# ariel415el/SoundEventDetection-Pytorch

Measured on AMD Instinct MI355X. Metric: SED train clips/sec (60s,64-mel,9-layer CNN), higher is better.
Workload: dtype bf16; 1 GPU; Cnn_AvgPooling main widths [32, 64, 128, 128], 60 s / 32 kHz / 64-mel clips (T=6001 frames, NFFT 1024, hop 320), batch 32/GPU, train step = waveform->log-mel->fwd->BCE->bwd->Adam-amsgrad; frontend_constants=bench, graph_replay=False, global_batch=32, frames=6001, parallelism=dp1, frontend_in_step=True, frontend_overlapped=False, frontend_overlap_mode=0, sync_bn=False, rccl_group=False, collectives_executed=False

## Files before the change

soundeventdetection-pytorch_amd/csrc/conv_common.h:

```cpp
#pragma once
#include "common.h"

#include <stdlib.h>

template <typename T> __device__ __forceinline__ int swz(int col);
template <> __device__ __forceinline__ int swz<bf16_t>(int col) { return ((col >> 2) & 3) << 3; }
template <> __device__ __forceinline__ int swz<float>(int col) { return col & 31; }

template <typename T> struct Raw8;
template <> struct Raw8<bf16_t> { bf16x8 v; };
template <> struct Raw8<float> { f32x4 a, b; };
template <typename T> __device__ __forceinline__ Raw8<T> raw_load8(const T* p);
template <> __device__ __forceinline__ Raw8<bf16_t> raw_load8<bf16_t>(const bf16_t* p) {
    Raw8<bf16_t> r; r.v = *reinterpret_cast<const bf16x8*>(p); return r;
}
template <> __device__ __forceinline__ Raw8<float> raw_load8<float>(const float* p) {
    Raw8<float> r;
    r.a = *reinterpret_cast<const f32x4*>(p);
    r.b = *reinterpret_cast<const f32x4*>(p + 4);
    return r;
}
__device__ __forceinline__ void raw_to_f(const Raw8<bf16_t>& r, float (&v)[8]) {
#pragma unroll
    for (int i = 0; i < 8; ++i) v[i] = (float)r.v[i];
}
__device__ __forceinline__ void raw_to_f(const Raw8<float>& r, float (&v)[8]) {
#pragma unroll
    for (int i = 0; i < 4; ++i) { v[i] = r.a[i]; v[4 + i] = r.b[i]; }
}

typedef __attribute__((ext_vector_type(4))) unsigned u32x4;
typedef __attribute__((ext_vector_type(2))) unsigned u32x2;
#define SED_OOB 0x80000000u

__device__ __forceinline__ __amdgpu_buffer_rsrc_t make_srd(const void* base, size_t bytes) {
    return __builtin_amdgcn_make_buffer_rsrc(const_cast<void*>(base), 0, (int)(bytes > 0xFFFFFFFFull ? 0xFFFFFFFFu : (unsigned)bytes),
                                             0x00020000);
}
template <typename T> __device__ __forceinline__ Raw8<T> buf_load8(__amdgpu_buffer_rsrc_t r, unsigned voff);
template <> __device__ __forceinline__ Raw8<bf16_t> buf_load8<bf16_t>(__amdgpu_buffer_rsrc_t r, unsigned voff) {
    Raw8<bf16_t> o;
    o.v = __builtin_bit_cast(bf16x8, __builtin_amdgcn_raw_buffer_load_b128(r, voff, 0, 0));
    return o;
}
template <> __device__ __forceinline__ Raw8<float> buf_load8<float>(__amdgpu_buffer_rsrc_t r, unsigned voff) {
    Raw8<float> o;
    o.a = __builtin_bit_cast(f32x4, __builtin_amdgcn_raw_buffer_load_b128(r, voff, 0, 0));
    o.b = __builtin_bit_cast(f32x4, __builtin_amdgcn_raw_buffer_load_b128(r, voff + 16, 0, 0));
    return o;
}
template <typename T> __device__ __forceinline__ void buf_store8(__amdgpu_buffer_rsrc_t r, unsigned voff, const float (&v)[8]);
template <> __device__ __forceinline__ void buf_store8<bf16_t>(__amdgpu_buffer_rsrc_t r, unsigned voff, const float (&v)[8]) {
    bf16x8 a;
#pragma unroll
    for (int i = 0; i < 8; ++i) a[i] = (bf16_t)v[i];
    __builtin_amdgcn_raw_buffer_store_b128(__builtin_bit_cast(u32x4, a), r, voff, 0, 0);
}
template <> __device__ __forceinline__ void buf_store8<float>(__amdgpu_buffer_rsrc_t r, unsigned voff, const float (&v)[8]) {
    f32x4 a, b;
#pragma unroll
    for (int i = 0; i < 4; ++i) { a[i] = v[i]; b[i] = v[4 + i]; }
    __builtin_amdgcn_raw_buffer_store_b128(__builtin_bit_cast(u32x4, a), r, voff, 0, 0);
    __builtin_amdgcn_raw_buffer_store_b128(__builtin_bit_cast(u32x4, b), r, voff + 16, 0, 0);
}
template <typename T> __device__ __forceinline__ void buf_store4(__amdgpu_buffer_rsrc_t r, unsigned voff, const float (&v)[4]);
template <> __device__ __forceinline__ void buf_store4<bf16_t>(__amdgpu_buffer_rsrc_t r, unsigned voff, const float (&v)[4]) {
    bf16x4 a;
#pragma unroll
    for (int i = 0; i < 4; ++i) a[i] = (bf16_t)v[i];
    __builtin_amdgcn_raw_buffer_store_b64(__builtin_bit_cast(u32x2, a), r, voff, 0, 0);
}
template <> __device__ __forceinline__ void buf_store4<float>(__amdgpu_buffer_rsrc_t r, unsigned voff, const float (&v)[4]) {
    f32x4 a;
#pragma unroll
    for (int i = 0; i < 4; ++i) a[i] = v[i];
    __builtin_amdgcn_raw_buffer_store_b128(__builtin_bit_cast(u32x4, a), r, voff, 0, 0);
}
template <typename T> __device__ __forceinline__ void buf_load4(__amdgpu_buffer_rsrc_t r, unsigned voff, float (&v)[4]);
template <> __device__ __forceinline__ void buf_load4<bf16_t>(__amdgpu_buffer_rsrc_t r, unsigned voff, float (&v)[4]) {
    const bf16x4 a = __builtin_bit_cast(bf16x4, __builtin_amdgcn_raw_buffer_load_b64(r, voff, 0, 0));
#pragma unroll
    for (int i = 0; i < 4; ++i) v[i] = (float)a[i];
}
template <> __device__ __forceinline__ void buf_load4<float>(__amdgpu_buffer_rsrc_t r, unsigned voff, float (&v)[4]) {
    const f32x4 a = __builtin_bit_cast(f32x4, __builtin_amdgcn_raw_buffer_load_b128(r, voff, 0, 0));
#pragma unroll
    for (int i = 0; i < 4; ++i) v[i] = a[i];
}
template <typename T> __device__ __forceinline__ void lds_store_raw(T* dst, const Raw8<T>& r);
template <> __device__ __forceinline__ void lds_store_raw<bf16_t>(bf16_t* dst, const Raw8<bf16_t>& r) {
    *reinterpret_cast<bf16x8*>(dst) = r.v;
}
template <> __device__ __forceinline__ void lds_store_raw<float>(float* dst, const Raw8<float>& r) {
    *reinterpret_cast<f32x4*>(dst) = r.a;
    *reinterpret_cast<f32x4*>(dst + 4) = r.b;
}

template <typename T, int W, int ROWS, int WP, int NTHR, int PS>
struct HaloPlan {
    static constexpr int ITEMS = ROWS * (W + 2) * 4;
    static constexpr int IPT = (ITEMS + NTHR - 1) / NTHR;
    unsigned voff[IPT];
    int lds[IPT];
    unsigned colmask;
    Raw8<T> raw[IPT];

    __device__ __forceinline__ void init(int tid, int Cinp) {
        const int cq = tid & 3;
        colmask = 0;
#pragma unroll
        for (int u = 0; u < IPT; ++u) {
            const int it = tid + u * NTHR;
            const int pix = it >> 2;
            const int rowi = pix / (W + 2), coli = pix - rowi * (W + 2);
            const bool ok = (it < ITEMS) && coli >= 1 && coli <= W;
            voff[u] = ok ? (unsigned)(((rowi * W + coli) * Cinp + cq * 8) * (int)sizeof(T)) : SED_OOB;
            if (ok) colmask |= 1u << u;
            if constexpr (sizeof(T) == 2) lds[u] = (rowi * WP + coli) * PS + ((PS == 32) ? ((cq * 8) ^ swz<T>(coli)) : cq * 8);
            else lds[u] = (rowi * WP + coli) * PS;
        }
    }
    __device__ __forceinline__ void issue(__amdgpu_buffer_rsrc_t img, unsigned tile_off) {
#pragma unroll
        for (int u = 0; u < IPT; ++u) raw[u] = buf_load8<T>(img, voff[u] + tile_off);
    }
    template <int PRO>
    __device__ __forceinline__ void commit(T* __restrict__ xs, int tid, const float* __restrict__ pro_scale,
                                           const float* __restrict__ pro_shift, int c0, int row_lo, int row_hi) const {
        const int cq = tid & 3;
        float sc[8], sh[8];
        if (PRO == SED_PRO_BNRELU) {
#pragma unroll
            for (int e = 0; e < 8; ++e) { sc[e] = pro_scale[c0 + cq * 8 + e]; sh[e] = pro_shift[c0 + cq * 8 + e]; }
        }
        const bool boundary = (row_lo > 0) || (row_hi < ROWS - 1);
#pragma unroll
        for (int u = 0; u < IPT; ++u) {
            const int it = tid + u * NTHR;
            if (u == IPT - 1 && it >= ITEMS) break;
            if constexpr (sizeof(T) == 2) {
                if (PRO == SED_PRO_NONE) {
                    lds_store_raw<T>(xs + lds[u], raw[u]);
                } else {
                    float v[8];
                    raw_to_f(raw[u], v);
                    bool keep = (colmask >> u) & 1;
                    if (boundary) {
                        const int rowi = (it >> 2) / (W + 2);
                        keep = keep && rowi >= row_lo && rowi <= row_hi;
                    }
#pragma unroll
                    for (int e = 0; e < 8; ++e) v[e] = keep ? fmaxf(0.f, fmaf(v[e], sc[e], sh[e])) : 0.f;
                    store8<T>(xs + lds[u], v);
                }
            } else {
                float v[8];
                raw_to_f(raw[u], v);
                const int pix = it >> 2;
                const int rowi = pix / (W + 2), coli = pix - rowi * (W + 2);
                const bool keep = ((colmask >> u) & 1) && rowi >= row_lo && rowi <= row_hi;
                if (PRO == SED_PRO_BNRELU) {
#pragma unroll
                    for (int e = 0; e < 8; ++e) v[e] = keep ? fmaxf(0.f, fmaf(v[e], sc[e], sh[e])) : 0.f;
                }
                const int sx = swz<T>(coli);
#pragma unroll
                for (int e = 0; e < 8; ++e) xs[lds[u] + ((cq * 8 + e) ^ sx)] = v[e];
            }
        }
    }
};


typedef __attribute__((ext_vector_type(4))) short s16x4;
typedef __attribute__((ext_vector_type(8))) short s16x8;
__device__ __forceinline__ s16x4 ds_read_tr16_b64(const bf16_t* p) {
    typedef __attribute__((address_space(3))) s16x4 lds_s16x4;
    return __builtin_amdgcn_ds_read_tr16_b64_v4i16((lds_s16x4*)(const __attribute__((address_space(3))) void*)p);
}
__device__ __forceinline__ bf16x8 join_tr(const s16x4& lo, const s16x4& hi) {
    return __builtin_bit_cast(bf16x8, __builtin_shufflevector(lo, hi, 0, 1, 2, 3, 4, 5, 6, 7));
}


#ifndef SED_BOUNDARY_BRANCH
#define SED_BOUNDARY_BRANCH 1
#endif

enum { DZ_GIVEN = 0, DZ_POOL = 1, DZ_BN = 2 };

struct Wgrad2Params {
    const void* x;
    const float* pro_scale;
    const float* pro_shift;
    const void* dz;
    const void* zsrc;
    const float* scale;
    const float* shift;
    const float* ca;
    const float* cb;
    const float* cc;
    void* dz_out;
    float* ws;
    int B, H, Cinp, Coutp;
    int tilesPerImg, totalTiles, tpb, strips;
    int pro, pool;
    const float* c1_x;
    const float* c1_mean;
    const float* c1_std;
    const float* c1_w;
    int dbg;
    unsigned tpi_M, tpi_l;
    int dzexp;
};


int wgrad3_strips(int B, int H, int W, int Cinp, int Coutp);
int launch_wgrad3(int dzmode, Wgrad2Params& p, int W, hipStream_t st);
int wgrad_wide_strips(int B, int H, int W, int Cinp, int Coutp);
int launch_wgrad_wide(int dzmode, Wgrad2Params& p, int W, hipStream_t st);
int reduce_wgrad_slabs(const float* ws, float* dwpack, int slabs, size_t n, float* dw, int Cout, int Cin, int Cinp, int Coutp, hipStream_t st);

static inline bool sed_w_specialised(int W) { return W == 8 || W == 16 || W == 32 || W == 64; }

#ifdef SED_DEBUG_SWITCHES
#define SED_DBG(p, bit) ((p).dbg & (bit))
#define SED_SET_PRIO(x) set_wave_prio(x)
#else
#define SED_DBG(p, bit) 0
#define SED_SET_PRIO(x) ((void)0)
#endif
static inline int sed_dbg_env() { const char* d = sed_getenv("SED_DBG"); return d ? atoi(d) : 0; }

__device__ __forceinline__ void set_wave_prio(int pr) {
    switch (pr & 3) {
        case 1: __builtin_amdgcn_s_setprio(1); break;
        case 2: __builtin_amdgcn_s_setprio(2); break;
        case 3: __builtin_amdgcn_s_setprio(3); break;
        default: break;
    }
}


struct ConvParams {
    const void* x;
    const float* pro_scale;
    const float* pro_shift;
    const void* wpack;
    void* z;
    const void* zref;
    const float* epi_scale;
    const float* epi_shift;
    const float* epi_mean;
    const float* epi_invstd;
    float* partial;
    int B, H, Cinp, Coutp;
    int tilesPerImg, totalTiles, tpb, nparts;
    int pro, epi;
    int wres;
    const float* c1_x;
    const float* c1_mean;
    const float* c1_std;
    const float* c1_w;
    void* c1_mask;
    int dbg;
    int col_only;
    const unsigned char* cnt;
    int* flag;
    int dry;
    const void* dz_g;
    const float* dz_ca;
    const float* dz_cb;
    const float* dz_cc;
    const float* dz_sc;
    const float* dz_sh;
    void* dz_out;
    int dz_pool;
    unsigned tpi_M, tpi_l, nch_M, nch_l;
    int xexp;
};
inline void sed_fastdiv_make(unsigned d, unsigned* M, unsigned* l) {
    unsigned ll = 0;
    while ((1ull << ll) < d) ++ll;
    *l = ll;
    *M = (unsigned)((((1ull << ll) - d) << 32) / d + 1);
}
__device__ __forceinline__ int sed_fastdiv(int n, unsigned M, unsigned l) { return (int)((__umulhi((unsigned)n, M) + (unsigned)n) >> l); }

int launch_conv_x3(int half, ConvParams& p, int W, hipStream_t st);
int launch_conv_x3pc(ConvParams& p, int W, hipStream_t st);
int launch_wgrad_x3pc(int dzmode, Wgrad2Params& p, int W, hipStream_t st);
int launch_wgrad_x3(int half, int dzmode, Wgrad2Params& p, int W, int wn, hipStream_t st);

int launch_conv_anyw(int dtype, ConvParams& p, int W, hipStream_t st);
int launch_wgrad_anyw(int dtype, int dzmode, Wgrad2Params& p, int W, hipStream_t st);

int launch_conv_pc(ConvParams& p, int W, hipStream_t st);
int launch_conv_wir(ConvParams& p, int W, hipStream_t st);
int launch_conv_w4(ConvParams& p, int W, hipStream_t st);

struct BwdFusedParams {
    const void* x;
    const float* pro_scale;
    const float* pro_shift;
    const void* gsrc;
    const void* zsrc;
    const float* scale;
    const float* shift;
    const float* ca;
    const float* cb;
    const float* cc;
    const void* wpack_t;
    void* dx;
    const void* zref;
    const unsigned char* cnt;
    const float* epi_scale;
    const float* epi_shift;
    const float* epi_mean;
    const float* epi_invstd;
    float* partial;
    int* flag;
    float* ws;
    int B, H, Cinp, Coutp;
    int pool, dzmode, pro, epi;
    int nparts, nwg, tilesPerImg, totalTiles, tpb;
    int dry;
    int prio;
    int abl;
};
int bwd_fused_nwg(int B, int H, int W, int Cinp, int Coutp, int dzmode, int pro, int epi);
int launch_bwd_fused(BwdFusedParams& p, int W, hipStream_t st);
int bwd_fused_max_nwg(int B, int H, int W, int Cinp, int Coutp);
int bwd_fused_c1_nwg(int B, int H);
int bwd_fused_cs_nstrips(int B, int H, int W, int Cinp, int Coutp, int dzmode, int pro, int epi, int pool);
int launch_bwd_fused_cs(BwdFusedParams& p, int W, hipStream_t st);

int launch_bwd_fused_c1(const float* x1, const float* fmean, const float* fstd, const float* w1, const float* sc1, const float* sh1,
                        const void* dy, const void* z2, const float* sc2, const float* sh2, const float* ca, const float* cb,
                        const float* cc, const void* wpack_t, float* a_part, int nparts, float* ws, int B, int H,
                        int* nwg, hipStream_t st);

enum { SED_PRO_C1 = 2, SED_EPI_RELUBWD_C1 = 3 };
enum { SED_PRO_DZBN = 11, SED_PRO_DZPOOL = 12 };

struct C1Ctx {
    float w[9][8];
    float mu[3], is[3];
};
__device__ __forceinline__ void c1ctx_init(C1Ctx& c, const float* __restrict__ w1, int ch0, const float* __restrict__ fmean,
                                           const float* __restrict__ fstd, int col, int W) {
#pragma unroll
    for (int k = 0; k < 9; ++k)
#pragma unroll
        for (int e = 0; e < 8; ++e) c.w[k][e] = w1[(ch0 + e) * 9 + k];
#pragma unroll
    for (int j = 0; j < 3; ++j) {
        const int cc = col + j - 1;
        const bool ok = cc >= 0 && cc < W;
        c.mu[j] = (ok && fmean) ? fmean[cc] : 0.f;
        c.is[j] = ok ? (fstd ? 1.0f / fstd[cc] : 1.0f) : 0.f;
    }
}
__device__ __forceinline__ void c1_norm_row(const C1Ctx& c, const float (&raw)[3], bool row_ok, float (&xn)[3]) {
#pragma unroll
    for (int j = 0; j < 3; ++j) xn[j] = row_ok ? (raw[j] - c.mu[j]) * c.is[j] : 0.f;
}
__device__ __forceinline__ void c1_eval(const C1Ctx& c, const float (&r0)[3], const float (&r1)[3], const float (&r2)[3],
                                        float (&z)[8]) {
#pragma unroll
    for (int e = 0; e < 8; ++e) z[e] = 0.f;
#pragma unroll
    for (int j = 0; j < 3; ++j)
#pragma unroll
        for (int e = 0; e < 8; ++e) z[e] = fmaf(r0[j], c.w[j][e], z[e]);
#pragma unroll
    for (int j = 0; j < 3; ++j)
#pragma unroll
        for (int e = 0; e < 8; ++e) z[e] = fmaf(r1[j], c.w[3 + j][e], z[e]);
#pragma unroll
    for (int j = 0; j < 3; ++j)
#pragma unroll
        for (int e = 0; e < 8; ++e) z[e] = fmaf(r2[j], c.w[6 + j][e], z[e]);
}
__device__ __forceinline__ float buf_load_f32(__amdgpu_buffer_rsrc_t r, unsigned voff) {
    return __builtin_bit_cast(float, __builtin_amdgcn_raw_buffer_load_b32(r, voff, 0, 0));
}

struct C1Mma {
    bf16x8 wa;
};
__device__ __forceinline__ void c1mma_init(C1Mma& m, const float* __restrict__ w1, const float* __restrict__ scale,
                                           const float* __restrict__ shift, int lane) {
    const int ch = lane & 31, g = lane >> 5;
    const float sc = scale[ch], sh = shift[ch];
    const bf16_t sh_hi = (bf16_t)sh;
    const bf16_t sh_lo = (bf16_t)(sh - (float)sh_hi);
#pragma unroll
    for (int j = 0; j < 8; ++j) {
        const int row = 2 * g + (j >> 2), dx = j & 3;
        m.wa[j] = (row < 3 && dx < 3) ? (bf16_t)(w1[ch * 9 + 3 * row + dx] * sc) : (row == 3 && dx == 0) ? sh_hi : (row == 3 && dx == 1) ? sh_lo : (bf16_t)0.f;
    }
}
template <int XW>
__device__ __forceinline__ bf16x8 c1mma_patch_f(const float* __restrict__ xt, int rr, int half, int lane) {
    const int col = half * 32 + (lane & 31), g = lane >> 5;
    const float* p0 = xt + (rr + 2 * g) * XW + col;
    float v[8];
#pragma unroll
    for (int t = 0; t < 3; ++t) { v[t] = p0[t]; v[4 + t] = p0[XW + t]; }
    v[3] = 0.f; v[7] = 0.f;
    bf16x8 xb;
#pragma unroll
    for (int j = 0; j < 8; ++j) xb[j] = (bf16_t)v[j];
    u32x4 xw = __builtin_bit_cast(u32x4, xb);
    xw[2] = g ? 0x3F803F80u : xw[2];
    xw[3] = g ? 0u : xw[3];
    return __builtin_bit_cast(bf16x8, xw);
}
typedef unsigned c1_u32x2_a4 __attribute__((ext_vector_type(2), aligned(4)));
template <int W, int R>
struct C1Tile {
    static constexpr int XP = W + 8;
    static constexpr int XB = ((R * XP / 2 + 15) / 32 * 32 + 16) * 2 >= R * XP ? ((R * XP / 2 + 15) / 32 * 32 + 16) * 2 : ((R * XP / 2 + 15) / 32 * 32 + 48) * 2;
    static constexpr int N = XB + R * XP;
    static_assert(XB >= R * XP && (XB / 2) % 32 == 16 && XP % 2 == 0, "copy B offset");
};
template <int W, int R>
__device__ __forceinline__ void c1tile_lane_offsets(int half, int lane, int& o1, int& o2) {
    typedef C1Tile<W, R> TL;
    const int p = half * 32 + (lane & 31), g = lane >> 5;
    const int src = (p & 1) ? TL::XB + p - 1 : p;
    o1 = src + (g ? 2 * TL::XP : 0);
    o2 = g ? TL::XP + W + 4 : TL::XP + src;
}
__device__ __forceinline__ bf16x8 c1mma_patch_b(const bf16_t* __restrict__ row_rr, int o1, int o2) {
    const c1_u32x2_a4 lo = *reinterpret_cast<const c1_u32x2_a4*>(row_rr + o1);
    const c1_u32x2_a4 hi = *reinterpret_cast<const c1_u32x2_a4*>(row_rr + o2);
    const u32x4 xw = {lo[0], lo[1], hi[0], hi[1]};
    return __builtin_bit_cast(bf16x8, xw);
}
template <int W, int R>
__device__ __forceinline__ void c1tile_init(bf16_t* __restrict__ t, int tid, int nthr) {
    typedef C1Tile<W, R> TL;
    unsigned* w = reinterpret_cast<unsigned*>(t);
    for (int i = tid; i < TL::N / 2; i += nthr) {
        const int e = 2 * i, r = e / TL::XP, c = e - r * TL::XP;
        w[i] = (e < R * TL::XP && c == W + 4) ? 0x3F803F80u : 0u;
    }
}
template <int W, int R>
__device__ __forceinline__ void c1tile_store(bf16_t* __restrict__ t, int r, int c, float x) {
    typedef C1Tile<W, R> TL;
    const bf16_t b = (bf16_t)x;
    t[r * TL::XP + c] = b;
    if (c >= 1) t[TL::XB + r * TL::XP + c - 1] = b;
}
template <int XW, bool WANT_MASK>
__device__ __forceinline__ void c1mma_block(const C1Mma& m, const float* __restrict__ xt, int rr, int half, int lane,
                                            float (&a)[16], unsigned& mask) {
    const bf16x8 xb = c1mma_patch_f<XW>(xt, rr, half, lane);
    f32x16 d;
#pragma unroll
    for (int i = 0; i < 16; ++i) d[i] = 0.f;
    d = __builtin_amdgcn_mfma_f32_32x32x16_bf16(m.wa, xb, d, 0, 0, 0);
    mask = 0;
#pragma unroll
    for (int i = 15; i >= 0; --i) {
        const float y = d[i];
        a[i] = fmaxf(0.f, y);
        if (WANT_MASK)
            asm volatile("v_cmp_lt_f32 vcc, 0, %1\n\tv_addc_co_u32 %0, vcc, %0, %0, vcc" : "+v"(mask) : "v"(y) : "vcc");
    }
}

template <int XW>
__device__ __forceinline__ f32x16 c1mma_block_mfma(const C1Mma& m, const float* __restrict__ xt, int rr, int half, int lane) {
    const bf16x8 xb = c1mma_patch_f<XW>(xt, rr, half, lane);
    f32x16 d;
#pragma unroll
    for (int i = 0; i < 16; ++i) d[i] = 0.f;
    return __builtin_amdgcn_mfma_f32_32x32x16_bf16(m.wa, xb, d, 0, 0, 0);
}
__device__ __forceinline__ f32x16 c1mma_block_mfma_b(const C1Mma& m, const bf16_t* __restrict__ row_rr, int o1, int o2) {
    const bf16x8 xb = c1mma_patch_b(row_rr, o1, o2);
    f32x16 d;
#pragma unroll
    for (int i = 0; i < 16; ++i) d[i] = 0.f;
    return __builtin_amdgcn_mfma_f32_32x32x16_bf16(m.wa, xb, d, 0, 0, 0);
}
template <bool WANT_MASK>
__device__ __forceinline__ void c1mma_block_tail_pk(const f32x16& d, unsigned (&w)[8], unsigned& mask) {
    unsigned mlo = 0, mhi = 0;
    const unsigned one2 = 0x00010001u;
#pragma unroll
    for (int k = 0; k < 8; ++k) {
        const f32x2 r = {d[2 * k], d[2 * k + 1]};
        const bf16x2 rb = __builtin_convertvector(r, bf16x2);
        sed_i16x2 ri = __builtin_bit_cast(sed_i16x2, rb);
        ri = __builtin_elementwise_max(ri, (sed_i16x2){0, 0});
        w[k] = __builtin_bit_cast(unsigned, ri);
        if (WANT_MASK) {
            unsigned t;
            asm("v_pk_min_u16 %0, %1, %2" : "=v"(t) : "v"(w[k]), "v"(one2));
            const unsigned wt = (1u << ((2 * k) & 7)) | (1u << (16 + ((2 * k + 1) & 7)));
            if (k < 4) mlo = __builtin_amdgcn_udot4(t, wt, mlo, false);
            else mhi = __builtin_amdgcn_udot4(t, wt, mhi, false);
        }
    }
    mask = mlo | (mhi << 8);
}
template <bool WANT_MASK>
__device__ __forceinline__ void c1mma_block_tail(const C1Mma& m, const f32x16& d, float (&a)[16], unsigned& mask) {
    mask = 0;
#pragma unroll
    for (int i = 15; i >= 0; --i) {
        const float y = d[i];
        a[i] = fmaxf(0.f, y);
        if (WANT_MASK)
            asm volatile("v_cmp_lt_f32 vcc, 0, %1\n\tv_addc_co_u32 %0, vcc, %0, %0, vcc" : "+v"(mask) : "v"(y) : "vcc");
    }
}
```

soundeventdetection-pytorch_amd/csrc/sed_conv_pc.hip:

```cpp
#include "conv_common.h"

#include <stdlib.h>


namespace {

#ifdef SED_STAMPS
constexpr bool kStamps = true;
#else
constexpr bool kStamps = false;
#endif

constexpr int kPcBlocks = 256;

__device__ __forceinline__ void wg_barrier() {
    asm volatile("s_waitcnt lgkmcnt(0)\n\ts_barrier" ::: "memory");
}

__device__ __forceinline__ int xswz(int col) { return (col >> 2) & 3; }
__device__ __forceinline__ f32x16 zero16() {
    f32x16 z;
#pragma unroll
    for (int i = 0; i < 16; ++i) z[i] = 0.f;
    return z;
// ... 791 lines not shown
        constexpr bool WREGS = C1PRO && NT == 1 && !COL && SED_PC_WREGS;
        bf16x8 wreg[WREGS ? 18 : 1];
        if constexpr (WREGS) {
            const T* __restrict__ wgl = reinterpret_cast<const T*>(p.wpack);
#pragma unroll
            for (int k = 0; k < 18; ++k) {
                const int tap = k >> 1, ks = k & 1;
                wreg[k] = *reinterpret_cast<const bf16x8*>(wgl + ((size_t)(tap * 4 + ks * 2 + hh) * Coutp + n0 + r) * 8);
            }
        }
        auto compute = [&](const T* __restrict__ xsb, const T* __restrict__ wsc, bool first) {
            if (SED_DBG(p, 2)) return;
            if constexpr (WREGS) {
                bf16x8 xf[3][2];
                auto ldx = [&](int k, bf16x8 (&xd)[2]) {
                    const int tap = k >> 1, ks = k & 1, ti = tap / 3, tj = tap % 3;
#pragma unroll
                    for (int mt = 0; mt < 2; ++mt)
                        xd[mt] = *reinterpret_cast<const bf16x8*>(xsb + xoff[mt][tj][ks] + (ti * WP + tj) * 32);
                };
                ldx(0, xf[0]);
                ldx(1, xf[1]);
#pragma unroll
                for (int k = 0; k < 18; ++k) {
                    if (k + 2 < 18) ldx(k + 2, xf[(k + 2) % 3]);
                    __builtin_amdgcn_sched_barrier(0);
#pragma unroll
                    for (int mt = 0; mt < 2; ++mt) acc[mt][0] = mfma(wreg[k], xf[k % 3][mt], acc[mt][0]);
                    __builtin_amdgcn_sched_barrier(0);
                }
                return;
            }
            constexpr int RD = 3;
            bf16x8 xf[RD][2], wf[RD][NT];
            auto ld = [&](int k, bf16x8 (&xd)[2], bf16x8 (&wd)[NT]) {
                const int tap = k >> 1, ks = k & 1, ti = tap / 3, tj = tap % 3;
#pragma unroll
                for (int mt = 0; mt < 2; ++mt)
                    xd[mt] = *reinterpret_cast<const bf16x8*>(xsb + xoff[mt][tj][ks] + (ti * WP + tj) * 32);
#pragma unroll
                for (int nt = 0; nt < NT; ++nt)
                    wd[nt] = *reinterpret_cast<const bf16x8*>(wsc + woff + ((tap * 4 + ks * 2) * BN + nt * 32) * 8);
            };
            constexpr int NK = COL ? 6 : 18;
            auto kmap = [](int s2) { return COL ? (s2 >> 1) * 6 + 2 + (s2 & 1) : s2; };
#pragma unroll
            for (int k = 0; k < RD - 1 && k < NK; ++k) ld(kmap(k), xf[k], wf[k]);
#pragma unroll
            for (int k = 0; k < NK; ++k) {
                if (k + RD - 1 < NK) ld(kmap(k + RD - 1), xf[(k + RD - 1) % RD], wf[(k + RD - 1) % RD]);
                __builtin_amdgcn_sched_barrier(0);
#pragma unroll
                for (int nt = 0; nt < NT; ++nt)
#pragma unroll
                    for (int mt = 0; mt < 2; ++mt) {
                        if (SED_PC_ZEROC && k == 0) {
                            if (first) { asm volatile("" ::: "memory"); acc[mt][nt] = mfma(wf[k % RD][nt], xf[k % RD][mt], zero16()); }
                            else acc[mt][nt] = mfma(wf[k % RD][nt], xf[k % RD][mt], acc[mt][nt]);
                        } else {
                            acc[mt][nt] = mfma(wf[k % RD][nt], xf[k % RD][mt], acc[mt][nt]);
                        }
                    }
                __builtin_amdgcn_sched_barrier(0);
            }
        };

        if (C1PRO && !BLD) build_c1(0, wave, std::integral_constant<int, 0>{});

        unsigned long long tc[4] = {0, 0, 0, 0};
        auto stamp = [&]() -> unsigned long long { return kStamps ? __builtin_amdgcn_s_memtime() : 0ull; };
        auto citer = [&](int j, const T* __restrict__ xsb) {
            const unsigned long long c0 = stamp();
            wg_barrier();
            const unsigned long long c1 = stamp();
            tc[0] += c1 - c0;
            if (C1PRO && j >= nst) return;
            if (j >= nst) return;
            if constexpr (kSplitBuild) build_c1_issue(j + 1, wave);
            constexpr bool ONECH = C1PRO && SED_PC_ONECH;
            const int tl = ONECH ? j : DIV_NCH(j), kc = ONECH ? 0 : j - tl * nchunks;
            if (ONECH || (!SED_PC_ZEROC && kc == 0)) {
#pragma unroll
                for (int mt = 0; mt < 2; ++mt)
#pragma unroll
                    for (int nt = 0; nt < NT; ++nt)
#pragma unroll
                        for (int i = 0; i < 16; ++i) acc[mt][nt][i] = 0.f;
            }
            compute(xsb, ws + (wres ? kc : (j & 1)) * WS, kc == 0);
            const unsigned long long c2 = stamp();
            tc[1] += c2 - c1;
            if (!ONECH && kc != nchunks - 1) return;
            T* osb = os + (nos == 2 ? (tl & 1) : 0) * OSZ;
            if (!(SED_DBG(p, 128)))
#pragma unroll
            for (int mt = 0; mt < 2; ++mt)
#pragma unroll
                for (int nt = 0; nt < NT; ++nt)
#pragma unroll
                    for (int g = 0; g < 4; ++g) {
                        float v[4];
#pragma unroll
                        for (int e = 0; e < 4; ++e) v[e] = acc[mt][nt][4 * g + e];
                        store4<T>(osb + ostg[mt] + nt * 32 + 8 * g, v);
                    }
            const unsigned long long c3 = stamp();
            if constexpr (kSplitBuild) build_c1_finish(j + 1, wave);
            else if (C1PRO && !BLD) build_c1(j + 1, wave, std::integral_constant<int, C1SHARE ? (SED_C1_SHARE == 2 ? 3 : 1) : 0>{});
            if constexpr (CSTAT) {
                const int tile = t_begin + tl;
                const int b_ = DIV_TPI(tile), h0_ = (tile - b_ * p.tilesPerImg) * TH;
                bf16x8 ones;
#pragma unroll
                for (int e = 0; e < 8; ++e) ones[e] = (bf16_t)1.0f;
#pragma unroll
                for (int mt = 0; mt < 2; ++mt) {
                    const int q0s = (wave * 2 + mt) * 32;
                    if (h0_ + q0s / W < H) {
#pragma unroll
                        for (int ks = 0; ks < 2; ++ks) {
                            const T* fp = osb + (q0s + 16 * ks) * BNP;
                            const bf16x8 f = join_tr(ds_read_tr16_b64(fp + offS[0]), ds_read_tr16_b64(fp + offS[1]));
                            gacc = mfma(f, f, gacc);
                            sacc = mfma(ones, f, sacc);
                        }
                    }
                }
            }
            if (kStamps) { tc[2] += c3 - c2; tc[3] += stamp() - c3; }
        };
        for (int j = 0; j < NI; j += 2) {
            citer(j, xs0);
            citer(j + 1, xs0 + XS);
        }
        if (kStamps && (SED_DBG(p, 16)) && blockIdx.x == 8 && lane == 0 && wave == 1)
            printf("pc consumer wave %d: %d stages; cycles barrier %llu kloop %llu staging %llu c1build %llu\n", wave, NI, tc[0], tc[1], tc[2], tc[3]);
        if constexpr (CSTAT) {
            const int idx = 4 * (r >> 3) + (r & 3);
            float dg = 0.f;
#pragma unroll
            for (int i = 0; i < 16; ++i) dg = (i == idx) ? gacc[i] : dg;
            S[0] = sacc[0];
            Q[0] = dg;
        }
        }
    }

    if (EPI != SED_EPI_STORE) {
        __syncthreads();
        float* red = reinterpret_cast<float*>(smem);
        if constexpr (CSTAT) {
            if (wave < 4) {
                const int r_ = lane & 31, hh_ = lane >> 5;
                if (hh_ == 0) red[(wave * 2 + 0) * 32 + r_] = S[0];
                if (hh_ == ((r_ >> 2) & 1)) red[(wave * 2 + 1) * 32 + r_] = Q[0];
            }
        } else
        if (wave >= 4 && wave < 4 + NPW) {
            const int pt = tid - 256;
#pragma unroll
            for (int e = 0; e < 8; ++e) { red[pt * 16 + e] = S[e]; red[pt * 16 + 8 + e] = Q[e]; }
        }
        __syncthreads();
        if (tid < 2 * BN) {
            const int stat = tid / BN, cn = tid % BN;
            const int cg = cn >> 3, e = cn & 7;
            float tot = 0.f;
            if constexpr (CSTAT) {
                for (int w = 0; w < 4; ++w) tot += red[(w * 2 + stat) * 32 + cn];
            } else
            for (int k = 0; k < FQS; ++k) tot += red[(cg + IPR * k) * 16 + stat * 8 + e];
            if (EPI == SED_EPI_RELUBWD && stat) tot *= p.epi_invstd[n0 + cn];
            if constexpr (PSTATS) {
                float sraw = tot;
                if (stat) {
                    sraw = 0.f;
                    for (int k = 0; k < FQS; ++k) sraw += red[(cg + IPR * k) * 16 + e];
                }
                const float sc = p.epi_scale[n0 + cn], is = p.epi_invstd[n0 + cn];
                const float beta = fmaf(p.epi_mean[n0 + cn], sc, p.epi_shift[n0 + cn]);
                const bool ill = fabsf(beta) * is > 8.0f * fabsf(sc);
                if (!stat) {
                    tot = 0.25f * sraw;
                } else if (sc != 0.f && !ill) {
                    tot = (tot - 0.25f * beta * sraw) * (is / sc);
                } else {
                    if (tot != 0.f || sraw != 0.f) atomicOr(p.flag, 1);
                    tot = 0.f;
                }
            }
            p.partial[((size_t)bx * 2 + stat) * Coutp + n0 + cn] = tot;
            for (int row = bx + nbx; row < p.nparts; row += nbx) p.partial[((size_t)row * 2 + stat) * Coutp + n0 + cn] = 0.f;
        }
    }
}

template <int W, int BN, int PRO, int EPI, bool COL = false, int NPW = 4, bool BLD = false, bool WR = false>
int launch_pc_n(ConvParams& p, hipStream_t st) {
    constexpr int BM = 256, TH = BM / W, ROWS = TH + 2, WP = (W + 2 + 3) & ~3;
    const int nchunks = p.Cinp / 32;
    const int nos = nchunks == 1 ? 2 : 1;
    auto lds_for = [&](int wbufs_) -> size_t {
        return ((size_t)2 * ROWS * WP * 32 + (size_t)(WR ? 0 : wbufs_) * 9 * 32 * BN + (size_t)nos * BM * (BN + 8)) * sizeof(bf16_t) +
               (size_t)((PRO == SED_PRO_DZBN || PRO == SED_PRO_DZPOOL) ? 5 : 2) * p.Cinp * sizeof(float) +
               (PRO == SED_PRO_C1 ? (size_t)2 * C1Tile<W, ROWS + 2>::N * sizeof(bf16_t) : 0);
    };
    p.wres = (WR || nchunks <= 2 || lds_for(nchunks) <= 160 * 1024) ? 1 : 0;
    const size_t lds = lds_for(p.wres ? nchunks : 2);
    if (lds > 160 * 1024) return -1;
    if (p.dry) return 0;
    if (int rc_ = sed_set_max_lds<&conv_pc_kernel<W, BN, PRO, EPI, COL, NPW, BLD, WR>>(lds)) return rc_;
    p.tilesPerImg = cdiv(p.H, TH);
    p.totalTiles = p.B * p.tilesPerImg;
    sed_fastdiv_make((unsigned)p.tilesPerImg, &p.tpi_M, &p.tpi_l);
    sed_fastdiv_make((unsigned)nchunks, &p.nch_M, &p.nch_l);
    const int ny = p.Coutp / BN;
    long long blocks = kPcBlocks;
    if (const char* e = sed_getenv("SED_CONV_BLOCKS")) blocks = atoll(e) > 0 ? atoll(e) : blocks;
    int nbx = (int)(blocks / ny);
    if (nbx > p.nparts) nbx = p.nparts;
    if (nbx > p.totalTiles) nbx = p.totalTiles;
    if (nbx < 1) nbx = 1;
    p.tpb = cdiv(p.totalTiles, nbx);
    conv_pc_kernel<W, BN, PRO, EPI, COL, NPW, BLD, WR><<<dim3(nbx * ny), dim3(256 + 64 * NPW + (BLD ? 256 : 0)), lds, st>>>(p);
    return 0;
}

template <int W, int BN, int PRO, int EPI, bool COL = false, bool WR = false>
int launch_pc(ConvParams& p, hipStream_t st) {
    if constexpr (WR) {
        return launch_pc_n<W, BN, PRO, EPI, COL, 4, false, true>(p, st);
    } else {
#ifdef SED_EXPERIMENTS
    if constexpr (PRO == SED_PRO_C1 && BN == 32) {
        const char* e = sed_getenv("SED_PC_BUILDERS");
        if (e && e[0] == '1') return launch_pc_n<W, BN, PRO, EPI, COL, 4, true>(p, st);
        if (e && e[0] == '2') return launch_pc_n<W, BN, PRO, EPI, COL, 8, true>(p, st);
        if (e && e[0] == '3') return launch_pc_n<W, BN, PRO, EPI, COL, 8, false>(p, st);
    }
    constexpr bool can8 = EPI != SED_EPI_RELUBWD_C1 && !(EPI == SED_EPI_RELUBWD && BN == 64) && PRO != SED_PRO_C1;
    if constexpr (can8) {
        const char* e = sed_getenv("SED_PC_PROD");
        if (e && e[0] == '8') return launch_pc_n<W, BN, PRO, EPI, COL, 8>(p, st);
    }
#endif
    return launch_pc_n<W, BN, PRO, EPI, COL, 4>(p, st);
    }
}

template <int W, int BN, bool COL = false, bool WR = false>
int dispatch_pc_pe(ConvParams& p, hipStream_t st) {
    if (p.pro == SED_PRO_NONE && p.epi == SED_EPI_STATS) return launch_pc<W, BN, SED_PRO_NONE, SED_EPI_STATS, COL, WR>(p, st);
    if (p.pro == SED_PRO_BNRELU && p.epi == SED_EPI_STATS) return launch_pc<W, BN, SED_PRO_BNRELU, SED_EPI_STATS, COL, WR>(p, st);
    if (p.pro == SED_PRO_NONE && p.epi == SED_EPI_STORE) return launch_pc<W, BN, SED_PRO_NONE, SED_EPI_STORE, COL, WR>(p, st);
    if (p.pro == SED_PRO_BNRELU && p.epi == SED_EPI_STORE) return launch_pc<W, BN, SED_PRO_BNRELU, SED_EPI_STORE, COL, WR>(p, st);
    if (p.pro == SED_PRO_NONE && p.epi == SED_EPI_RELUBWD) return launch_pc<W, BN, SED_PRO_NONE, SED_EPI_RELUBWD, COL, WR>(p, st);
    if constexpr (!COL) {
        if (p.pro == SED_PRO_NONE && p.epi == SED_EPI_POOLSTATS) return launch_pc<W, BN, SED_PRO_NONE, SED_EPI_POOLSTATS, COL, WR>(p, st);
    }
#ifdef SED_EXPERIMENTS
    if constexpr (!COL && (W == 16 || W == 8) && BN >= 64) {
        if (p.pro == SED_PRO_DZBN && p.epi == SED_EPI_POOLSTATS) return launch_pc<W, BN, SED_PRO_DZBN, SED_EPI_POOLSTATS, COL, WR>(p, st);
        if (p.pro == SED_PRO_DZBN && p.epi == SED_EPI_STORE) return launch_pc<W, BN, SED_PRO_DZBN, SED_EPI_STORE, COL, WR>(p, st);
        if (p.pro == SED_PRO_DZPOOL && p.epi == SED_EPI_RELUBWD) return launch_pc<W, BN, SED_PRO_DZPOOL, SED_EPI_RELUBWD, COL, WR>(p, st);
    }
#endif
    return -1;
}

int dispatch_pc_c1(ConvParams& p, hipStream_t st) {
    if (p.pro == SED_PRO_C1 && p.Cinp == 32) {
        if (p.Coutp % 64 == 0) {
            if (p.epi == SED_EPI_STATS) return launch_pc<64, 64, SED_PRO_C1, SED_EPI_STATS>(p, st);
            if (p.epi == SED_EPI_STORE) return launch_pc<64, 64, SED_PRO_C1, SED_EPI_STORE>(p, st);
        } else {
            if (p.epi == SED_EPI_STATS) return launch_pc<64, 32, SED_PRO_C1, SED_EPI_STATS>(p, st);
            if (p.epi == SED_EPI_STORE) return launch_pc<64, 32, SED_PRO_C1, SED_EPI_STORE>(p, st);
        }
    }
    if (p.pro == SED_PRO_NONE && p.epi == SED_EPI_RELUBWD_C1 && p.Coutp == 32)
        return launch_pc<64, 32, SED_PRO_NONE, SED_EPI_RELUBWD_C1>(p, st);
    return -1;
}

template <int W>
int dispatch_pc_bn(ConvParams& p, hipStream_t st) {
    if constexpr (W <= 32) {
        const char* ew = sed_getenv("SED_PC_WR");
        if (!(ew && ew[0] == '0')) {
            if (p.Coutp % 128 == 0 && p.Cinp >= 96) return dispatch_pc_pe<W, 128, false, true>(p, st);
        }
    }
    const char* e = sed_getenv("SED_PC_BN");
    const bool slim = e ? (e[0] == '3') : false;
    if (p.Coutp % 64 == 0 && !(slim && p.Cinp >= 128)) return dispatch_pc_pe<W, 64>(p, st);
    return dispatch_pc_pe<W, 32>(p, st);
}

}

int launch_conv_pc(ConvParams& p, int W, hipStream_t st) {
    if (p.Cinp % 32 || p.Coutp % 32 || p.Cinp > 512) return -1;
    if (p.pro == SED_PRO_C1 || p.epi == SED_EPI_RELUBWD_C1) return W == 64 ? dispatch_pc_c1(p, st) : -1;
    switch (W) {
        case 8: {
            const char* e = sed_getenv("SED_PC_W8");
            if (e && e[0] == '0') return -1;
            if (p.col_only) return (p.Coutp % 64 == 0) ? dispatch_pc_pe<8, 64, true>(p, st) : dispatch_pc_pe<8, 32, true>(p, st);
            return dispatch_pc_bn<8>(p, st);
        }
        case 16: return dispatch_pc_bn<16>(p, st);
        case 32: return dispatch_pc_bn<32>(p, st);
        case 64: return dispatch_pc_bn<64>(p, st);
    }
    return -1;
}
```

Before: 7935 clips/s.

## Add warp-specialized conv kernel with DMA producer waves for narrow 128-channel layers

Adds a new 768-thread conv kernel for W=16/8, Cin 64/128, Cout 128 layers. Four waves issue buffer-to-LDS DMA into a triple-buffered input ring and run the epilogue (ReLU-backward / pool statistics) for the previous tile, while eight waves run the MFMA k-loop with register-prefetched weights. An LDS atomic counter hands off the staging buffer between the two groups. It is routed first from launch_conv_pc, by default only for the two Cin=128 cases chosen (W16 RELUBWD, W8 POOLSTATS), and risks spin-wait and LDS-capacity occupancy costs.

```diff
diff --git a/soundeventdetection-pytorch_amd/csrc/conv_aw_map.h b/soundeventdetection-pytorch_amd/csrc/conv_aw_map.h
--- /dev/null
+++ b/soundeventdetection-pytorch_amd/csrc/conv_aw_map.h
@@ -0,0 +1,37 @@
+#pragma once
+
+#if defined(__HIPCC__) || defined(__CUDACC__)
+#define SED_AW_HD __host__ __device__ __forceinline__
+#else
+#define SED_AW_HD inline
+#endif
+
+namespace sed_aw {
+
+SED_AW_HD constexpr int xswz(int col) { return (col >> 2) & 3; }
+
+template <int W>
+struct Geo {
+    static constexpr int BM = 256, TH = BM / W, ROWS = TH + 2, WP = (W + 2 + 3) & ~3;
+    static constexpr int SLOTS = ROWS * WP * 4;
+    static constexpr int NDMA = (SLOTS + 63) / 64;
+    static constexpr int XSTRIDE = NDMA * 1024;
+};
+
+struct DmaSrc {
+    bool valid;
+    int row, col;
+    int gslot;
+};
+template <int W>
+SED_AW_HD constexpr DmaSrc dma_src(int sl) {
+    const int pix = sl >> 2, s = sl & 3;
+    const int row = pix / Geo<W>::WP, col = pix - row * Geo<W>::WP;
+    return DmaSrc{row < Geo<W>::ROWS && col >= 1 && col <= W, row, col, s ^ xswz(col)};
+}
+template <int W>
+SED_AW_HD constexpr int frag_slot(int prow, int pcol, int ti, int tj, int ks, int hh) {
+    return ((prow + ti) * Geo<W>::WP + pcol + tj) * 4 + ((ks * 2 + hh) ^ xswz(pcol + tj));
+}
+
+}
diff --git a/soundeventdetection-pytorch_amd/csrc/conv_common.h b/soundeventdetection-pytorch_amd/csrc/conv_common.h
--- a/soundeventdetection-pytorch_amd/csrc/conv_common.h
+++ b/soundeventdetection-pytorch_amd/csrc/conv_common.h
@@ -296,6 +296,7 @@
 int launch_wgrad_anyw(int dtype, int dzmode, Wgrad2Params& p, int W, hipStream_t st);
 
 int launch_conv_pc(ConvParams& p, int W, hipStream_t st);
+int launch_conv_aw(ConvParams& p, int W, hipStream_t st);
 int launch_conv_wir(ConvParams& p, int W, hipStream_t st);
 int launch_conv_w4(ConvParams& p, int W, hipStream_t st);
 
diff --git a/soundeventdetection-pytorch_amd/csrc/sed_conv_aw.hip b/soundeventdetection-pytorch_amd/csrc/sed_conv_aw.hip
--- /dev/null
+++ b/soundeventdetection-pytorch_amd/csrc/sed_conv_aw.hip
@@ -0,0 +1,431 @@
+#include "conv_common.h"
+#include "conv_aw_map.h"
+
+#include <stdlib.h>
+#include <type_traits>
+
+namespace {
+
+constexpr int kAwBlocks = 256;
+
+#ifdef SED_STAMPS
+constexpr bool kAwStamps = true;
+#else
+constexpr bool kAwStamps = false;
+#endif
+
+typedef __attribute__((address_space(3))) char aw_lds_char;
+
+__device__ __forceinline__ void aw_barrier() {
+    asm volatile("s_waitcnt lgkmcnt(0)\n\ts_barrier" ::: "memory");
+}
+template <int N>
+__device__ __forceinline__ void aw_wait_vm() {
+    asm volatile("s_waitcnt vmcnt(%0)" ::"n"(N) : "memory");
+}
+__device__ __forceinline__ void aw_dma16(__amdgpu_buffer_rsrc_t srd, unsigned dst, unsigned voff) {
+    unsigned keep;
+    asm volatile("s_mov_b32 %0, m0\n\ts_mov_b32 m0, %2\n\ts_nop 0\n\tbuffer_load_dwordx4 %1, %3, 0 offen lds\n\ts_mov_b32 m0, %0"
+                 : "=&s"(keep)
+                 : "v"(voff), "s"(dst), "s"(srd)
+                 : "memory");
+}
+
+template <int I> using IC = std::integral_constant<int, I>;
+
+template <int W, int CIN, int BN, int EPI>
+__global__ __launch_bounds__(768) void conv_aw_kernel(ConvParams p) {
+    typedef bf16_t T;
+    typedef sed_aw::Geo<W> G;
+    constexpr int BM = G::BM, TH = G::TH, WP = G::WP;
+    constexpr int NCH = CIN / 32;
+    constexpr int NFP = NCH;
+    constexpr int BNP = BN + 8, OSZ = BM * BNP;
+    constexpr int NCT = BN / 32, PG = 8 / NCT, MT = 8 / PG;
+    constexpr int NDMA = G::NDMA, DMAX = (NDMA + 3) / 4, DMIN = NDMA / 4;
+    constexpr int NP = 256, IPR = BN / 8, FIPT = BM * IPR / NP, FQS = NP / IPR;
+    constexpr bool RELUBWD = EPI == SED_EPI_RELUBWD, PSTATS = EPI == SED_EPI_POOLSTATS, ZREF = RELUBWD || PSTATS;
+    constexpr int ZB = (FIPT + NFP - 1) / NFP;
+    static_assert(BN == 128 && NCT == 4 && MT == 4, "one 32-channel tile x 128 pixels per wave");
+    static_assert(NCH == 2 || NCH == 4, "64 / 128 input channels");
+    static_assert(FIPT == 16 && FIPT % 4 == 0, "epilogue items");
+
+    extern __shared__ __attribute__((aligned(16))) char smem[];
+    T* os = reinterpret_cast<T*>(smem + 3 * G::XSTRIDE);
+    float* pcoef = reinterpret_cast<float*>(os + OSZ);
+    int* os_free = reinterpret_cast<int*>(pcoef + 3 * BN);
+    const unsigned xs_lds = (unsigned)(size_t)(aw_lds_char*)smem;
+
+    const int H = p.H, Coutp = p.Coutp;
+    const int tid = threadIdx.x, lane = tid & 63, wave = __builtin_amdgcn_readfirstlane(tid >> 6);
+    const unsigned logical = xcd_remap(blockIdx.x, gridDim.x);
+    const int bx = (int)logical, nbx = (int)gridDim.x;
+    const T* __restrict__ wg = reinterpret_cast<const T*>(p.wpack);
+    const T* __restrict__ xg = reinterpret_cast<const T*>(p.x);
+    T* __restrict__ zg = reinterpret_cast<T*>(p.z);
+    const T* __restrict__ zr = reinterpret_cast<const T*>(p.zref);
+    constexpr unsigned wchunk_bytes = 36u * BN * 8 * 2;
+    const size_t ximg_ = (size_t)H * W * CIN, zimg_ = (size_t)H * W * BN;
+
+    const int t_begin = bx * p.tpb;
+    const int t_end = min(p.totalTiles, t_begin + p.tpb);
+    const int ntl = t_end > t_begin ? t_end - t_begin : 0;
+
+    if (RELUBWD) {
+        for (int i = tid; i < 3 * BN; i += 768) {
+            const int rowc = i / BN, c = i - rowc * BN;
+            pcoef[i] = rowc == 0 ? p.epi_scale[c] : rowc == 1 ? p.epi_shift[c] : p.epi_mean[c];
+        }
+    }
+    if (tid == 0) *os_free = 0;
+    __syncthreads();
+
+    const int lw = wave & 3;
+    unsigned dvoff[DMAX];
+#pragma unroll
+    for (int i = 0; i < DMAX; ++i) {
+        const sed_aw::DmaSrc s = sed_aw::dma_src<W>(((i * 4 + lw) << 6) + lane);
+        dvoff[i] = s.valid ? (unsigned)(((s.row * W + s.col) * CIN + s.gslot * 8) * 2) : SED_OOB;
+    }
+    auto tile_pos = [&](int tl, int& b, int& h0) {
+        const int tile = t_begin + tl;
+        b = sed_fastdiv(tile, p.tpi_M, p.tpi_l);
+        h0 = (tile - b * p.tilesPerImg) * TH;
+    };
+    auto dma_stage = [&](int bi, int b, int h0, int kc) {
+        const __amdgpu_buffer_rsrc_t xsrd = make_srd(xg + (size_t)b * ximg_, ximg_ * 2);
+        const unsigned xt = (unsigned)((((h0 - 1) * W - 1) * CIN + kc * 32) * 2);
+        const unsigned dst = xs_lds + (unsigned)bi * G::XSTRIDE + (unsigned)lw * 1024u;
+#pragma unroll
+        for (int i = 0; i < DMAX; ++i)
+            if (i < DMIN || i * 4 + lw < NDMA) aw_dma16(xsrd, dst + i * 4096u, dvoff[i] + xt);
+    };
+
+    const int r = lane & 31, hh = lane >> 5;
+    const int ct = wave & 3, pg = wave >> 2;
+    const int q0 = pg * MT * 32 + r, prow0 = q0 / W, pcol0 = q0 % W;
+    int xoff[3][2];
+#pragma unroll
+    for (int tj = 0; tj < 3; ++tj)
+#pragma unroll
+        for (int ks = 0; ks < 2; ++ks) xoff[tj][ks] = sed_aw::frag_slot<W>(prow0, pcol0, 0, tj, ks, hh) * 8;
+    constexpr int DMT = (32 / W) * WP * 32;
+    const int ostg0 = q0 * BNP + ct * 32 + 4 * hh;
+    const unsigned wvoff = (unsigned)(((hh * BN + ct * 32 + r) * 8) * 2);
+    constexpr unsigned wkstep = BN * 32;
+    f32x16 acc[MT];
+    constexpr int DA = 9;
+    bf16x8 wa[DA];
+    auto wld = [&](bool live, int kc, int k) -> bf16x8 {
+        const __amdgpu_buffer_rsrc_t srd = make_srd(wg, live ? (size_t)wchunk_bytes * NCH : 0);
+        return __builtin_bit_cast(bf16x8, __builtin_amdgcn_raw_buffer_load_b128(srd, wvoff, (unsigned)kc * wchunk_bytes + (unsigned)k * wkstep, 0));
+    };
+    auto compute = [&](auto c_c, const T* __restrict__ xsb, bool live_n) {
+        constexpr int C = decltype(c_c)::value, C_N = (C + 1 < NCH) ? C + 1 : 0;
+        bf16x8 xf[2][MT];
+        auto ldx = [&](int k, bf16x8 (&xd)[MT]) {
+            const int tap = k >> 1, ks = k & 1, ti = tap / 3, tj = tap % 3;
+#pragma unroll
+            for (int mt = 0; mt < MT; ++mt)
+                xd[mt] = *reinterpret_cast<const bf16x8*>(xsb + xoff[tj][ks] + ti * WP * 32 + mt * DMT);
+        };
+        ldx(0, xf[0]);
+#pragma unroll
+        for (int k = 0; k < 18; ++k) {
+            if (k + 1 < 18) ldx(k + 1, xf[(k + 1) & 1]);
+            __builtin_amdgcn_sched_barrier(0);
+            const int slot = (C * 18 + k) % DA;
+#pragma unroll
+            for (int mt = 0; mt < MT; ++mt) acc[mt] = mfma(wa[slot], xf[k & 1][mt], acc[mt]);
+            if (k + DA < 18) wa[slot] = wld(true, C, k + DA);
+            else wa[slot] = wld(live_n, C_N, k + DA - 18);
+            __builtin_amdgcn_sched_barrier(0);
+        }
+    };
+
+    const int pt = tid & 255;
+    const int fcg = pt % IPR, fq0 = pt / IPR;
+    const unsigned fl_off0 = (unsigned)((fq0 * BN + fcg * 8) * 2);
+    float S[8], Q[8];
+#pragma unroll
+    for (int e = 0; e < 8; ++e) { S[e] = 0.f; Q[e] = 0.f; }
+    Raw8<T> zraw[ZREF ? ZB : 1];
+    u32x2 craw[PSTATS ? ZB : 1];
+    auto zload = [&](auto ulo_c, auto uhi_c, bool live, int b, int h0) {
+        constexpr int ulo = decltype(ulo_c)::value, uhi = decltype(uhi_c)::value;
+        if constexpr (ZREF) {
+            const size_t zimg = live ? zimg_ : 0;
+            const __amdgpu_buffer_rsrc_t rs = make_srd(zr + (size_t)b * zimg, zimg * 2);
+            const unsigned tq = (unsigned)(h0 * W * BN * 2);
+#pragma unroll
+            for (int u = ulo; u < uhi; ++u) zraw[u - ulo] = buf_load8<T>(rs, fl_off0 + (unsigned)(u * FQS * BN * 2) + tq);
+            if constexpr (PSTATS) {
+                const __amdgpu_buffer_rsrc_t cs = make_srd(p.cnt + (size_t)b * zimg, zimg);
+#pragma unroll
+                for (int u = ulo; u < uhi; ++u)
+                    craw[u - ulo] = __builtin_bit_cast(u32x2, __builtin_amdgcn_raw_buffer_load_b64(cs, (fl_off0 + (unsigned)(u * FQS * BN * 2) + tq) >> 1, 0, 0));
+            }
+        }
+    };
+    auto zproc = [&](auto ulo_c, auto uhi_c, int b, int h0) {
+        constexpr int ulo = decltype(ulo_c)::value, uhi = decltype(uhi_c)::value;
+        const __amdgpu_buffer_rsrc_t zs = make_srd(zg + (size_t)b * zimg_, zimg_ * 2);
+        const unsigned tq = (unsigned)(h0 * W * BN * 2);
+        float ces[8], cet[8], cem[8];
+        if constexpr (RELUBWD) {
+            const f32x4* pc = reinterpret_cast<const f32x4*>(pcoef);
+#pragma unroll
+            for (int hlf = 0; hlf < 2; ++hlf) {
+                const f32x4 a = pc[fcg * 2 + hlf], bb = pc[BN / 4 + fcg * 2 + hlf], c = pc[2 * (BN / 4) + fcg * 2 + hlf];
+#pragma unroll
+                for (int e = 0; e < 4; ++e) { ces[4 * hlf + e] = a[e]; cet[4 * hlf + e] = bb[e]; cem[4 * hlf + e] = c[e]; }
+            }
+        }
+#pragma unroll
+        for (int u = ulo; u < uhi; ++u) {
+            const int q = fq0 + u * FQS;
+            const bf16x8 raw = *reinterpret_cast<const bf16x8*>(os + q * BNP + fcg * 8);
+            const bool valid = h0 + q / W < H;
+            const unsigned off = fl_off0 + (unsigned)(u * FQS * BN * 2) + tq;
+            if constexpr (RELUBWD) {
+                float v[8], z[8];
+#pragma unroll
+                for (int e = 0; e < 8; ++e) v[e] = (float)raw[e];
+                raw_to_f(zraw[u - ulo], z);
+#pragma unroll
+                for (int e = 0; e < 8; ++e) {
+                    const float gate = (valid && fmaf(z[e], ces[e], cet[e]) > 0.f) ? v[e] : 0.f;
+                    v[e] = gate;
+                    S[e] += gate;
+                    Q[e] = fmaf(gate, z[e] - cem[e], Q[e]);
+                }
+                buf_store8<T>(zs, off, v);
+            } else {
+                if constexpr (PSTATS) {
+                    float ya[8];
+                    raw_to_f(zraw[u - ulo], ya);
+#pragma unroll
+                    for (int e = 0; e < 8; ++e) {
+                        const float dyv = (float)raw[e];
+                        const float cf = (float)((craw[u - ulo][e >> 2] >> (8 * (e & 3))) & 0xffu);
+                        S[e] = fmaf(dyv, cf, S[e]);
+                        Q[e] = fmaf(dyv, ya[e], Q[e]);
+                    }
+                }
+                if (EPI == SED_EPI_STATS && valid) {
+#pragma unroll
+                    for (int e = 0; e < 8; ++e) { const float f = (float)raw[e]; S[e] += f; Q[e] = fmaf(f, f, Q[e]); }
+                }
+                __builtin_amdgcn_raw_buffer_store_b128(__builtin_bit_cast(u32x4, raw), zs, off, 0, 0);
+            }
+        }
+    };
+    auto epi_part = [&](auto pi_c, int b, int h0) {
+        constexpr int PI = decltype(pi_c)::value;
+        zproc(IC<FIPT * PI / NFP>{}, IC<FIPT * (PI + 1) / NFP>{}, b, h0);
+    };
+    auto epi_preload = [&](auto pi_c, bool live, int b, int h0) {
+        constexpr int PI = decltype(pi_c)::value;
+        zload(IC<FIPT * PI / NFP>{}, IC<FIPT * (PI + 1) / NFP>{}, live, b, h0);
+    };
+
+    int cb = 0, ch0 = 0, nb = 0, nh0 = 0, pb = 0, ph0 = 0;
+    if (ntl > 0) tile_pos(0, cb, ch0);
+    if (ntl > 1) tile_pos(1, nb, nh0);
+    if (wave >= 8) {
+        if (ntl > 0) {
+            dma_stage(0, cb, ch0, 0);
+            dma_stage(1, cb, ch0, 1);
+        }
+        aw_wait_vm<0>();
+    } else {
+#pragma unroll
+        for (int k = 0; k < DA; ++k) wa[k] = wld(ntl > 0, 0, k);
+    }
+
+    int bi = 0;
+    unsigned long long tc[6] = {0, 0, 0, 0, 0, 0};
+    auto stamp = [&]() -> unsigned long long { return kAwStamps ? __builtin_amdgcn_s_memtime() : 0ull; };
+    const unsigned long long t_start = stamp();
+    auto next_tile = [&](int tl) {
+        pb = cb; ph0 = ch0;
+        cb = nb; ch0 = nh0;
+        if (tl + 2 < ntl) tile_pos(tl + 2, nb, nh0);
+    };
+    if (wave >= 8) {
+        auto stage = [&](auto c_c, int tl) {
+            constexpr int C = decltype(c_c)::value;
+            const bool live = tl < ntl;
+            const unsigned long long s0 = stamp();
+            aw_barrier();
+            const unsigned long long s1 = stamp();
+            bool issued;
+            {
+                constexpr int C2 = C + 2;
+                const int b2 = (bi == 0) ? 2 : bi - 1;
+                if constexpr (C2 < NCH) {
+                    issued = live;
+                    if (live) dma_stage(b2, cb, ch0, C2);
+                } else {
+                    issued = tl + 1 < ntl;
+                    if (issued) dma_stage(b2, nb, nh0, C2 - NCH);
+                }
+            }
+            const unsigned long long s2 = stamp();
+            if constexpr (C < NFP) {
+                if (tl >= 1) epi_part(IC<C>{}, pb, ph0);
+                if constexpr (C + 1 < NFP) epi_preload(IC<C + 1>{}, tl >= 1, pb, ph0);
+            }
+            if constexpr (C == NCH - 1) {
+                asm volatile("" ::: "memory");
+                if (tl >= 1 && lane == 0) __hip_atomic_fetch_add(os_free, 1, __ATOMIC_RELAXED, __HIP_MEMORY_SCOPE_WORKGROUP);
+                epi_preload(IC<0>{}, live, cb, ch0);
+            }
+            const unsigned long long s3 = stamp();
+            if (!issued) aw_wait_vm<0>();
+            else if (DMAX > DMIN && (DMAX - 1) * 4 + lw < NDMA) aw_wait_vm<DMAX>();
+            else aw_wait_vm<DMIN>();
+            if (kAwStamps) { tc[0] += s1 - s0; tc[1] += s2 - s1; tc[2] += s3 - s2; tc[5] += stamp() - s3; }
+            bi = (bi == 2) ? 0 : bi + 1;
+        };
+        for (int tl = 0; tl <= ntl; ++tl) {
+            stage(IC<0>{}, tl);
+            stage(IC<1>{}, tl);
+            if constexpr (NCH == 4) {
+                stage(IC<2>{}, tl);
+                stage(IC<3>{}, tl);
+            }
+            next_tile(tl);
+        }
+    } else {
+        auto stage = [&](auto c_c, int tl) {
+            constexpr int C = decltype(c_c)::value;
+            const unsigned long long s0 = stamp();
+            aw_barrier();
+            const unsigned long long s1 = stamp();
+            if (kAwStamps) tc[0] += s1 - s0;
+            if (tl < ntl) {
+                if constexpr (C == 0) {
+#pragma unroll
+                    for (int mt = 0; mt < MT; ++mt)
+#pragma unroll
+                        for (int i = 0; i < 16; ++i) acc[mt][i] = 0.f;
+                }
+                const bool live_n = (C + 1 < NCH) ? true : (tl + 1 < ntl);
+                compute(IC<C>{}, reinterpret_cast<const T*>(smem + bi * G::XSTRIDE), live_n);
+                const unsigned long long s4 = stamp();
+                if constexpr (C == NCH - 1) {
+                    while (__hip_atomic_load(os_free, __ATOMIC_RELAXED, __HIP_MEMORY_SCOPE_WORKGROUP) < 4 * tl) __builtin_amdgcn_s_sleep(1);
+                    asm volatile("" ::: "memory");
+#pragma unroll
+                    for (int mt = 0; mt < MT; ++mt)
+#pragma unroll
+                        for (int g = 0; g < 4; ++g) {
+                            float v[4];
+#pragma unroll
+                            for (int e = 0; e < 4; ++e) v[e] = acc[mt][4 * g + e];
+                            store4<T>(os + ostg0 + mt * 32 * BNP + 8 * g, v);
+                        }
+                }
+                if (kAwStamps) { tc[3] += s4 - s1; tc[4] += stamp() - s4; }
+            }
+            bi = (bi == 2) ? 0 : bi + 1;
+        };
+        for (int tl = 0; tl <= ntl; ++tl) {
+            stage(IC<0>{}, tl);
+            stage(IC<1>{}, tl);
+            if constexpr (NCH == 4) {
+                stage(IC<2>{}, tl);
+                stage(IC<3>{}, tl);
+            }
+        }
+    }
+
+    if (kAwStamps && (p.dbg & 16) && blockIdx.x == 8 && lane == 0 && (wave == 1 || wave == 9))
+        printf("aw wave %d: %d tiles x %d stages; cycles barrier %llu dma-issue %llu epilogue %llu kloop %llu staging %llu dma-wait %llu total %llu\n", wave, ntl,
+               NCH, tc[0], tc[1], tc[2], tc[3], tc[4], tc[5], stamp() - t_start);
+
+    aw_wait_vm<0>();
+    if (EPI != SED_EPI_STORE) {
+        __syncthreads();
+        float* red = reinterpret_cast<float*>(smem);
+        if (wave >= 8) {
+#pragma unroll
+            for (int e = 0; e < 8; ++e) { red[pt * 16 + e] = S[e]; red[pt * 16 + 8 + e] = Q[e]; }
+        }
+        __syncthreads();
+        if (tid < 2 * BN) {
+            const int stat = tid / BN, cn = tid % BN;
+            const int cg = cn >> 3, e = cn & 7;
+            float tot = 0.f;
+            for (int k = 0; k < FQS; ++k) tot += red[(cg + IPR * k) * 16 + stat * 8 + e];
+            if (EPI == SED_EPI_RELUBWD && stat) tot *= p.epi_invstd[cn];
+            if constexpr (PSTATS) {
+                float sraw = tot;
+                if (stat) {
+                    sraw = 0.f;
+                    for (int k = 0; k < FQS; ++k) sraw += red[(cg + IPR * k) * 16 + e];
+                }
+                const float sc = p.epi_scale[cn], is = p.epi_invstd[cn];
+                const float beta = fmaf(p.epi_mean[cn], sc, p.epi_shift[cn]);
+                const bool ill = fabsf(beta) * is > 8.0f * fabsf(sc);
+                if (!stat) {
+                    tot = 0.25f * sraw;
+                } else if (sc != 0.f && !ill) {
+                    tot = (tot - 0.25f * beta * sraw) * (is / sc);
+                } else {
+                    if (tot != 0.f || sraw != 0.f) atomicOr(p.flag, 1);
+                    tot = 0.f;
+                }
+            }
+            p.partial[((size_t)bx * 2 + stat) * Coutp + cn] = tot;
+            for (int row = bx + nbx; row < p.nparts; row += nbx) p.partial[((size_t)row * 2 + stat) * Coutp + cn] = 0.f;
+        }
+    }
+}
+
+template <int W, int CIN, int EPI>
+int launch_aw(ConvParams& p, hipStream_t st) {
+    typedef sed_aw::Geo<W> G;
+    constexpr int BN = 128;
+    constexpr size_t lds = (size_t)3 * G::XSTRIDE + (size_t)G::BM * (BN + 8) * sizeof(bf16_t) + (size_t)3 * BN * sizeof(float) + 16;
+    static_assert(lds <= 160 * 1024 && lds >= 256 * 16 * sizeof(float), "LDS budget (the statistics reduction reuses it)");
+    if (p.dry) return 0;
+    if (int rc_ = sed_set_max_lds<&conv_aw_kernel<W, CIN, BN, EPI>>(lds)) return rc_;
+    p.tilesPerImg = cdiv(p.H, G::TH);
+    p.totalTiles = p.B * p.tilesPerImg;
+    sed_fastdiv_make((unsigned)p.tilesPerImg, &p.tpi_M, &p.tpi_l);
+    long long blocks = kAwBlocks;
+    if (const char* e = sed_getenv("SED_CONV_BLOCKS")) blocks = atoll(e) > 0 ? atoll(e) : blocks;
+    int nbx = (int)blocks;
+    if (nbx > p.nparts) nbx = p.nparts;
+    if (nbx > p.totalTiles) nbx = p.totalTiles;
+    if (nbx < 1) nbx = 1;
+    p.tpb = cdiv(p.totalTiles, nbx);
+    conv_aw_kernel<W, CIN, BN, EPI><<<dim3(nbx), dim3(768), lds, st>>>(p);
+    return 0;
+}
+
+template <int W, int CIN>
+int dispatch_aw_epi(ConvParams& p, hipStream_t st) {
+    switch (p.epi) {
+        case SED_EPI_RELUBWD: return launch_aw<W, CIN, SED_EPI_RELUBWD>(p, st);
+        case SED_EPI_STATS: return launch_aw<W, CIN, SED_EPI_STATS>(p, st);
+        case SED_EPI_STORE: return launch_aw<W, CIN, SED_EPI_STORE>(p, st);
+        case SED_EPI_POOLSTATS: return launch_aw<W, CIN, SED_EPI_POOLSTATS>(p, st);
+    }
+    return -1;
+}
+
+}
+
+int launch_conv_aw(ConvParams& p, int W, hipStream_t st) {
+    if (p.pro != SED_PRO_NONE || p.col_only || p.Coutp != 128 || !(p.Cinp == 64 || p.Cinp == 128) || !(W == 16 || W == 8)) return -1;
+    const char* e = sed_getenv("SED_CONV_AW");
+    if (e && e[0] == '0') return -1;
+    const bool all = e && e[0] == 'a';
+    const bool measured = p.Cinp == 128 && ((W == 16 && p.epi == SED_EPI_RELUBWD) || (W == 8 && p.epi == SED_EPI_POOLSTATS));
+    if (!all && !measured) return -1;
+    if (W == 16) return p.Cinp == 128 ? dispatch_aw_epi<16, 128>(p, st) : dispatch_aw_epi<16, 64>(p, st);
+    return p.Cinp == 128 ? dispatch_aw_epi<8, 128>(p, st) : dispatch_aw_epi<8, 64>(p, st);
+}
diff --git a/soundeventdetection-pytorch_amd/csrc/sed_conv_pc.hip b/soundeventdetection-pytorch_amd/csrc/sed_conv_pc.hip
--- a/soundeventdetection-pytorch_amd/csrc/sed_conv_pc.hip
+++ b/soundeventdetection-pytorch_amd/csrc/sed_conv_pc.hip
@@ -1117,6 +1117,7 @@
 int launch_conv_pc(ConvParams& p, int W, hipStream_t st) {
     if (p.Cinp % 32 || p.Coutp % 32 || p.Cinp > 512) return -1;
     if (p.pro == SED_PRO_C1 || p.epi == SED_EPI_RELUBWD_C1) return W == 64 ? dispatch_pc_c1(p, st) : -1;
+    if (const int rc_aw = launch_conv_aw(p, W, st); rc_aw >= 0) return rc_aw;
     switch (W) {
         case 8: {
             const char* e = sed_getenv("SED_PC_W8");
```

Result: no change. 7993 clips/s, median of 6 (+0.7%).
